# MarToonLi/StableDiffusionEO

Hardware: AMD Instinct MI355X
Metric: 512x512 canny2image images/sec (20 DDIM steps); ms per UNet step reported alongside (higher is better)
Workload: dtype f16; 1 GPU; SD1.5 + ControlNet-canny 512x512, batch=1 per GPU (CFG pair fused, N=2), 20 DDIM steps + VAE decode, fp16 storage / fp32 accumulate (BASELINE configs[1]); model_config=sd15, ddim_steps=20, parallelism=dp1 (image index -> rank, RCCL all_gather of final latents), weights=seeded synthetic (no checkpoint in the container)

## Files before the change

### stablediffusioneo_amd/csrc/api_ops.hip

```cpp
#include <stdarg.h>

#include "../../include/sdeo.h"
#include "sdeo_internal.h"
#include "kernels.h"

namespace sdeo {

static thread_local std::string g_last_error;

void set_error(const std::string& msg) { g_last_error = msg; }

int fail(const char* fmt, ...) {
  char buf[1024];
  va_list ap;
  va_start(ap, fmt);
  vsnprintf(buf, sizeof(buf), fmt, ap);
  va_end(ap);
  g_last_error = buf;
  return 1;
}

}

using namespace sdeo;
// ... 112 lines not shown
  return 0;
}

int sdeo_conv2d_nhwc_f16(void* y, const void* x, const void* w_krsc, const float* bias, const float* bias2, const void* res,
                         int n, int h, int w, int cin, int cout, int ksize, int stride, int upsample2x, int act, float scale,
                         void* workspace, size_t workspace_bytes, void* stream) {
  const Fp8Arm arm = disarm_fp8();
  ConvGemm p;
  if (int rc = fill_conv(p, n, h, w, cin, cout, ksize, stride, upsample2x)) return rc;
  p.x = (const f16*)x; p.w = (const f16*)w_krsc; p.y = (f16*)y; p.bias = bias; p.bias2 = bias2; p.res = (const f16*)res;
  p.act = act; p.scale = scale; p.workspace = (float*)workspace; p.workspace_bytes = workspace_bytes;
  take_fp8(p, arm);
  return conv_gemm(p, S(stream));
}

size_t sdeo_conv2d_pad_workspace_bytes(int n, int h, int w, int cin, int cout, int ksize, int stride, int upsample2x, int pad_before,
                                       int pad_after) {
  ConvGemm p;
  if (fill_conv(p, n, h, w, cin, cout, ksize, stride, upsample2x, pad_before, pad_after)) return 0;
  return conv_gemm_workspace_bytes(p);
}

int sdeo_conv2d_pad_nhwc_f16(void* y, const void* x, const void* w_krsc, const float* bias, const float* bias2, const void* res,
                             int n, int h, int w, int cin, int cout, int ksize, int stride, int upsample2x, int pad_before, int pad_after,
                             int act, float scale, void* workspace, size_t workspace_bytes, void* stream) {
  const Fp8Arm arm = disarm_fp8();
  SDEO_CHECK(pad_before >= 0 && pad_after >= 0, "conv2d_pad: negative padding (%d, %d)", pad_before, pad_after);
  ConvGemm p;
  if (int rc = fill_conv(p, n, h, w, cin, cout, ksize, stride, upsample2x, pad_before, pad_after)) return rc;
  p.x = (const f16*)x; p.w = (const f16*)w_krsc; p.y = (f16*)y; p.bias = bias; p.bias2 = bias2; p.res = (const f16*)res;
// ... 196 lines not shown
```

### stablediffusioneo_amd/csrc/conv_gemm.hip

```cpp
#include <stdlib.h>

#include <array>
#include <map>

#include <type_traits>
#include <utility>

#include "conv_inl.h"

namespace sdeo {

template <int BM, int BN, int STAGES, bool UPS, bool WS, bool W8 = false, int KPB = 1, bool MX = false>
__global__ __launch_bounds__(WS ? 512 : 256) void conv_gemm_dma_kernel(const KP pp) {
  kernarg_warm<sizeof(KP)>();
  KP pl = pp;
  asm volatile("" : "+s"(pl.M), "+s"(pl.N), "+s"(pl.K), "+s"(pl.Hi), "+s"(pl.Wi), "+s"(pl.Cin), "+s"(pl.Wo),
               "+s"(pl.S), "+s"(pl.stride), "+s"(pl.pad), "+s"(pl.HoWo), "+s"(pl.ldx), "+s"(pl.ldw), "+s"(pl.nk),
               "+s"(pl.nk_per_split), "+s"(pl.tiles_m), "+s"(pl.tiles_n), "+s"(pl.n_fastest));
  const KP& p = pl;
  static_assert(!MX || (WS && !W8 && !UPS && KPB == 1), "the block-scaled fp8 path exists for the plain wave-specialised GEMM");
  constexpr int BK = 64, RPP = 32;
  constexpr int WRPP = W8 ? 64 : 32;
  constexpr int XP = BM / RPP, WP = (BN + WRPP - 1) / WRPP, L = XP + WP;
  constexpr int TM = BM / 2, TN = BN / 2, MI = TM / 16, NI = TN / 16;
// ... 137 lines not shown
  };
  const int ngroups = (nk + KPB - 1) / KPB;

  if constexpr (WS) {
    if (!do_mma) {
      if (nk > 0) {
#pragma unroll
        for (int s = 0; s < PF; ++s)
          if (s < nk) issue(s);
        for (int g = 0; g < ngroups; ++g) {
          retire(g);
          __builtin_amdgcn_s_barrier();
          refill(g);
        }
      }
      __builtin_amdgcn_s_barrier();
      return;
    }
  }

  const int frow = lane & 15, fq = lane >> 4;
  constexpr int g0 = 0;
  f32x4 acc[NI][MI];
#pragma unroll
  for (int i = 0; i < NI; ++i)
#pragma unroll
    for (int j = 0; j < MI; ++j) acc[i][j] = f32x4{0.f, 0.f, 0.f, 0.f};

  float2* lnsm = reinterpret_cast<float2*>(smem + STAGES * STAGE);
  const bool ln_lds = p.ln_stats != nullptr && p.splitk == 1;
// ... 212 lines not shown
  stamp(p, 3);
  if (dbg_on(p, 32)) return;
  static_assert(4 * epilogue_scratch_bytes(TN) <= STAGES * STAGE, "epilogue scratch");
  constexpr int SCR = (STAGES * STAGE / 4) & ~15;
  constexpr int NBLK = epilogue_blocks(TN, MI, SCR);
  char* scratch = smem + wave * SCR;
  epilogue<NI, MI, TM, TN, NBLK>(pe, acc, m0, n0, wm, wn, frow, fq, z, bpre, use_bpre, scratch, ln_lds ? lnsm + wm * TM : nullptr);
  if (pe.gn_out) {
    asm volatile("s_waitcnt lgkmcnt(0)" ::: "memory");
    __builtin_amdgcn_s_barrier();
    if (wm == 0) {
      const int bimg = m0 / pe.HoWo;
      gn_partials_finish<TN, 2>(pe, smem + 2 * wn * SCR, SCR, lane, bimg, (m0 - bimg * pe.HoWo) / BM, n0 + wn * TN);
    }
  }
  if (dbg_on(p, 64)) {
    stamp(p, 4);
    asm volatile("s_waitcnt vmcnt(0)" ::: "memory");
    stamp(p, 5);
  }
}

template <int BM, int BN, int BK, bool GENERIC>
__global__ __launch_bounds__(256) void conv_gemm_kernel(const KP pp) {
  kernarg_warm<sizeof(KP)>();
  const KP& p = pp;
  constexpr int CPR = BK / 8;
  constexpr int RPP = 256 / CPR;
  constexpr int XP = BM / RPP;
  constexpr int WP = BN / RPP;
// ... 132 lines not shown
#pragma unroll
        for (int i = 0; i < NI; ++i)
#pragma unroll
          for (int j = 0; j < MI; ++j)
            acc[i][j] = __builtin_amdgcn_mfma_f32_16x16x32_f16(wf[i], xf[j], acc[i][j], 0, 0, 0);
      }
      if (more) store_tile(cur ^ 1);
      __syncthreads();
    }
  }
  f32x4 nob[NI];
#pragma unroll
  for (int i = 0; i < NI; ++i) nob[i] = f32x4{0.f, 0.f, 0.f, 0.f};
  static_assert(4 * epilogue_scratch_bytes(TN) <= 2 * STAGE, "epilogue scratch");
  epilogue<NI, MI, TM, TN>(p, acc, m0, n0, wm, wn, frow, fq, z, nob, false, smem + wave * epilogue_scratch_bytes(TN));
}

__global__ __launch_bounds__(256) void splitk_reduce_kernel(const KP pp) {
  kernarg_warm<sizeof(KP)>();
  KP pl = pp;
  asm volatile("" : "+s"(pl.M), "+s"(pl.N), "+s"(pl.HoWo), "+s"(pl.ldy), "+s"(pl.ldres), "+s"(pl.ld_bias2), "+s"(pl.act),
               "+s"(pl.bias_per_row), "+s"(pl.splitk), "+s"(pl.res_rows));
  const KP& p = pl;
  const int64_t idx = (int64_t)blockIdx.x * 256 + threadIdx.x;
  const int n4 = p.N / 4;
  if (idx >= (int64_t)p.M * n4) return;
  const int m = (int)(idx / n4);
  const int n = (int)(idx - (int64_t)m * n4) * 4;
  f32x4 v = f32x4{0.f, 0.f, 0.f, 0.f};
  const float* src = p.ws + (size_t)m * p.N + n;
  const size_t zs = (size_t)p.M * p.N;
  f32x4 bv = f32x4{0.f, 0.f, 0.f, 0.f}, b2 = bv;
  f16x4 rv = f16x4{0, 0, 0, 0};
  if (p.bias) {
    if (p.bias_per_row) bv += p.bias[m];
    else bv = *reinterpret_cast<const f32x4*>(p.bias + n);
  }
  if (p.bias2) b2 = *reinterpret_cast<const f32x4*>(p.bias2 + (size_t)(m / p.HoWo) * p.ld_bias2 + n);
  if (p.res) rv = *reinterpret_cast<const f16x4*>(p.res + (size_t)res_row(p, m) * p.ldres + n);
  for (int z0 = 0; z0 < p.splitk; z0 += 8) {
    f32x4 t[8];
// ... 20 lines not shown
  } else if (p.act == 4) {
#pragma unroll
    for (int t = 0; t < 4; ++t) v[t] = fmaxf(v[t], 0.f);
  }
  v *= p.scale;
#pragma unroll
  for (int t = 0; t < 4; ++t) v[t] += (float)rv[t];
  if (p.y32) {
    *reinterpret_cast<f32x4*>(p.y32 + (size_t)m * p.ldy + n) = v;
  } else {
    f16x4 o;
#pragma unroll
    for (int t = 0; t < 4; ++t) o[t] = (f16)v[t];
    *reinterpret_cast<f16x4*>(p.y + (size_t)m * p.ldy + n) = o;
  }
}

template <typename K>
static int launch_k(K kernel, int smem, DeviceOnce* attr_done, const KP& kp, int tiles, hipStream_t stream, int threads = 256) {
  if (attr_done->need()) {
    SDEO_HIP(hipFuncSetAttribute(reinterpret_cast<const void*>(kernel), hipFuncAttributeMaxDynamicSharedMemorySize, smem));
    attr_done->mark();
  }
  hipLaunchKernelGGL(kernel, dim3(tiles, 1, kp.splitk), dim3(threads), smem, stream, kp);
  SDEO_HIP(hipGetLastError());
  return 0;
}

template <int BM, int BN, int ST, bool UPS, bool WS, bool W8 = false, int KPB = 1, bool MX = false>
static int launch_dma(const KP& kp, int tiles, hipStream_t stream) {
// ... 236 lines not shown
               "conv_gemm: fp8 weights need Cin %% 64 == 0 (Cin=%d), no folded upsample and 16-byte aligned rows (ldw=%d bytes)", p.Cin, p.ldw);
  pl = make_plan(p);
  SDEO_CHECK(!p.wscale || (kTiles[pl.tile].caps & CAP_W8), "conv_gemm: no fp8-weight plan for this shape");
  SDEO_CHECK(!p.mx_sx || (kTiles[pl.tile].caps & CAP_MX), "conv_gemm: no block-scaled fp8 plan for this shape");
  SDEO_CHECK(p.act != 3 || (pl.splitk == 1 && (kTiles[pl.tile].bn / 2) % 32 == 0), "conv_gemm: no GEGLU-capable plan");
  kp = KP{};
  kp.x = p.x; kp.w = p.w; kp.y = p.y; kp.y32 = p.y32; kp.bias = p.bias; kp.bias2 = p.bias2; kp.res = p.res;
  kp.ws = p.workspace;
  kp.M = p.M; kp.N = p.N; kp.K = p.K;
  kp.Hi = p.Hi; kp.Wi = p.Wi; kp.Cin = p.Cin; kp.Ho = p.Ho; kp.Wo = p.Wo; kp.S = p.S; kp.stride = p.stride; kp.pad = p.pad;
  kp.ups = p.ups; kp.HoWo = p.Ho * p.Wo;
  kp.ldx = p.ldx; kp.ldw = p.ldw; kp.ldy = p.ldy; kp.ldres = p.ldres; kp.ld_bias2 = p.ld_bias2;
  kp.res_rows = p.res_rows > 0 ? p.res_rows : p.M;
  kp.act = p.act; kp.bias_per_row = p.bias_per_row; kp.scale = p.scale;
  kp.wscale = p.wscale;
  if (p.mx_sx) {
    SDEO_CHECK(p.mx_sw && p.R == 1 && p.S == 1 && p.stride == 1 && !p.ups && !p.wscale && p.Cin % 64 == 0 && !p.bias_per_row,
               "conv_gemm: block-scaled fp8 operands go with a plain GEMM whose K is a multiple of 128");
    SDEO_CHECK(p.mx_ldsx >= p.K / 16 && p.mx_ldsw >= p.K / 16, "conv_gemm: scale rows too short (%d, %d < %d)", p.mx_ldsx, p.mx_ldsw, p.K / 16);
    kp.mx_sx = p.mx_sx; kp.mx_sw = p.mx_sw; kp.mx_ldsx = p.mx_ldsx; kp.mx_ldsw = p.mx_ldsw;
  }
  if (p.ln_stats) {
    SDEO_CHECK(p.ln_s && p.ln_strips >= 1 && p.ln_ld >= p.ln_strips && p.ln_c > 0, "conv_gemm: incomplete LayerNorm-fold arguments");
    SDEO_CHECK(!p.bias_per_row && !p.y32, "conv_gemm: the LayerNorm fold applies to row-major fp16 products only");
    kp.ln_stats = p.ln_stats; kp.ln_s = p.ln_s; kp.ln_strips = p.ln_strips; kp.ln_ld = p.ln_ld;
    kp.ln_invc = 1.0f / (float)p.ln_c; kp.ln_eps = p.ln_eps;
  }
  if (p.stats_out) {
    const int strips = pl.splitk == 1 ? cdiv(p.N, plan_tn(pl)) : 0;
    SDEO_CHECK(strips >= 1 && p.stats_ld >= strips && p.y && !p.y32 && p.act != 3,
// ... 19 lines not shown
    static const int epi = [] { const char* e = getenv("SDEO_EPI_COALESCE"); return e ? atoi(e) : 1; }();
    kp.coalesce = epi && p.y && !p.y32 && pl.splitk == 1 && !p.bias_per_row && p.N % (p.act == 3 ? 16 : 8) == 0 && p.ldy % 8 == 0 &&
                  (reinterpret_cast<uintptr_t>(p.y) & 15) == 0 &&
                  (!p.res || (p.ldres % 8 == 0 && (reinterpret_cast<uintptr_t>(p.res) & 15) == 0));
    SDEO_CHECK(!p.gn_out || kp.coalesce, "conv_gemm: GroupNorm partials need the LDS-transposed epilogue");
  }
  if (pl.splitk > 1) {
    const size_t need = (size_t)pl.splitk * p.M * p.N * sizeof(float);
    SDEO_CHECK(p.workspace && p.workspace_bytes >= need, "conv_gemm: split-K workspace too small (%zu < %zu)",
               p.workspace_bytes, need);
  }
  if (kTiles[pl.tile].kind == TK_HALO) SDEO_CHECK(halo_ok(p, kTiles[pl.tile]), "conv_gemm: halo plan on an ineligible problem");
  return 0;
}

static int dispatch(const Plan& pl, int ups, bool w8, const KP& kp, hipStream_t stream) {
  if (pl.tile < 0 || pl.tile >= kTileCount) return fail("conv_gemm: bad tile %d", pl.tile);
  const TileCfg& c = kTiles[pl.tile];
  const TileLaunch launch = kp.mx_sx ? c.mx : w8 ? c.w8 : ups ? c.ups : c.plain;
  if (!launch) return fail("conv_gemm: tile %d has no %s instantiation", pl.tile, kp.mx_sx ? "block-scaled fp8" : w8 ? "fp8-weight" : "folded-upsample");
  if (int rc = launch(kp, pl.tiles_m * pl.tiles_n, stream)) return rc;
  if (pl.splitk > 1) {
    const int64_t n = (int64_t)kp.M * (kp.N / 4);
    hipLaunchKernelGGL(splitk_reduce_kernel, dim3((unsigned)cdiv64(n, 256)), dim3(256), 0, stream, kp);
    SDEO_HIP(hipGetLastError());
  }
  return 0;
}

int conv_gemm(const ConvGemm& p0, hipStream_t stream) {
  if (p0.mx_sx)
    SDEO_CHECK(p0.K % 128 == 0 && p0.ldx % 16 == 0 && p0.ldw % 16 == 0 && p0.K == p0.Cin, "conv_gemm: block-scaled fp8 GEMM needs K %% 128 == 0 (K=%d, ldx=%d, ldw=%d)", p0.K, p0.ldx, p0.ldw);
  const ConvGemm p = mx_view(p0);
  Plan pl;
  KP kp{};
  if (int rc = prepare(p, pl, kp)) return rc;
  g_last_tile = pl.tile; g_last_splitk = pl.splitk;
  return dispatch(pl, p.ups, p.wscale != nullptr, kp, stream);
}
// ... 98 lines not shown
```

### stablediffusioneo_amd/csrc/conv_halo.hip

```cpp
#include "conv_inl.h"

namespace sdeo {

constexpr int halo_xbytes(int ph, int pw) { return ((ph + 2) * (pw + 2) + 31) / 32 * 32 * 128; }
constexpr int halo_wbytes(int bn) { return (bn + 31) / 32 * 32 * 128; }
constexpr int halo_stages(int ph, int pw, int bn, int tpb = 1) {
  const int s = (160 * 1024 - 2 * halo_xbytes(ph, pw)) / (tpb * halo_wbytes(bn));
  const int cap = tpb == 1 ? 8 : 4;
  return s > cap ? cap : s;
}

template <int PH, int PW, int BN, int NMW, int TPB = 1>
__global__ __launch_bounds__(NMW * 64 + 256) void conv3x3_halo_kernel(const KP pp) {
  kernarg_warm<sizeof(KP)>();
  KP pl = pp;
  asm volatile("" : "+s"(pl.M), "+s"(pl.N), "+s"(pl.Hi), "+s"(pl.Wi), "+s"(pl.Cin), "+s"(pl.ldx), "+s"(pl.ldw),
               "+s"(pl.nk_per_split), "+s"(pl.tiles_m), "+s"(pl.tiles_n));
  const KP& p = pl;
  constexpr int BM = PH * PW;
  constexpr int MI = BM / (16 * NMW), NI = BN / 16;
  constexpr int HWD = PW + 2, XREAL = (PH + 2) * HWD;
  constexpr int LXW = (XREAL + 31) / 32;
  constexpr int XBYTES = LXW * 32 * 128;
  constexpr int LW = (BN + 31) / 32;
// ... 91 lines not shown
      const bool xin = tap >= 1 && tap <= PF - 1 && cr + 1 < ncr;
      if (a == PF - 1) {
        if (xin) wait_vmcnt<(PF - 1) * LWS + LXW>();
        else wait_vmcnt<(PF - 1) * LWS>();
      } else {
        static_for<PF - 1>([&](auto A) {
          if (a == A.value) wait_vmcnt<A.value * LWS>();
        });
      }
      __builtin_amdgcn_s_barrier();
      if (dbg_on(p, 8)) { if (++tap == SPS) { tap = 0; ++cr; } continue; }
      if (tap == 0 && cr + 1 < ncr) issue_x((cr + 1) & 1);
      if (it + PF < lsteps) issue_w((it + PF) % WST);
      if (++tap == SPS) { tap = 0; ++cr; }
    }
    __builtin_amdgcn_s_barrier();
    return;
  }

  const int wave = wave_all;
  const int frow = lane & 15, fq = lane >> 4;
  f32x4 acc[NI][MI];
#pragma unroll
  for (int i = 0; i < NI; ++i)
#pragma unroll
    for (int j = 0; j < MI; ++j) acc[i][j] = f32x4{0.f, 0.f, 0.f, 0.f};

  constexpr bool BPRE = NI <= 5;
  f32x4 bpre[NI];
  const bool use_bpre = BPRE && p.bias && !p.bias_per_row && p.splitk == 1;
// ... 148 lines not shown
```

### stablediffusioneo_amd/csrc/conv_inl.h

```cpp
#pragma once
#include <utility>

#include "kernels.h"

namespace sdeo {

struct KP {
  const f16* x;
  const f16* w;
  f16* y;
  float* y32;
  const float* bias;
  const float* bias2;
  const f16* res;
  float* ws;
  int M, N, K;
  int Hi, Wi, Cin, Ho, Wo, S, stride, pad, ups;
  int HoWo;
  int ldx, ldw, ldy, ldres, ld_bias2;
  int res_rows;
  int act, bias_per_row;
  float scale;
  int nk, nk_per_split, splitk;
  int tiles_m, tiles_n;
  int dbg;
  int n_fastest;
  int coalesce;
  const float* ln_stats;
  const float* ln_s;
  int ln_strips, ln_ld;
  float ln_invc, ln_eps;
  const float* wscale;
  float* stats_out;
  int stats_ld;
  float* gn_out;
  int gn_cpg, gn_slots, gn_groups;
  const unsigned char* mx_sx;
  const unsigned char* mx_sw;
  int mx_ldsx, mx_ldsw;
};

#ifdef SDEO_DEBUG_KERNELS
__device__ __forceinline__ bool dbg_on(const KP& p, int bit) { return (p.dbg & bit) != 0; }
#else
__device__ __forceinline__ constexpr bool dbg_on(const KP&, int) { return false; }
#endif

constexpr int kStampWGs = 4096, kStampSlots = 16;
static __device__ unsigned long long g_stamps[kStampWGs * kStampSlots];
__device__ __forceinline__ void stamp_cycles(const KP& p, int slot) {
  if (dbg_on(p, 64) && threadIdx.x == 0) {
    const int wg = blockIdx.x + gridDim.x * blockIdx.z;
    if (wg < kStampWGs) g_stamps[wg * kStampSlots + slot] = __builtin_amdgcn_s_memtime();
  }
}
__device__ __forceinline__ void stamp(const KP& p, int slot) {
  if (dbg_on(p, 64) && threadIdx.x == 0) {
    const int wg = blockIdx.x + gridDim.x * blockIdx.z;
    if (wg < kStampWGs) g_stamps[wg * kStampSlots + slot] = __builtin_amdgcn_s_memrealtime();
  }
}

static __device__ __attribute__((aligned(256))) const unsigned int g_zero_page[64] = {0};

template <int BK>
__device__ __forceinline__ int swz_chunk(int row, int chunk) {
  if (BK == 64) return chunk ^ ((row >> 1) & 7);
  return chunk ^ (((row >> 3) & 1) * 3);
}

constexpr int epilogue_scratch_bytes(int tn) { return 16 * (tn * 4 + 16) + 32 * tn; }

__device__ __forceinline__ unsigned long long pin_u64(unsigned long long v) {
  unsigned lo = __builtin_amdgcn_readfirstlane((unsigned)v), hi = __builtin_amdgcn_readfirstlane((unsigned)(v >> 32));
  asm volatile("" : "+s"(lo), "+s"(hi));
// ... 464 lines not shown
```

### stablediffusioneo_amd/csrc/handle_common.h

```cpp
#pragma once
#include <stdlib.h>

#include <algorithm>
#include <functional>
#include <string>
#include <unordered_map>
#include <vector>

#include "kernels.h"

namespace sdeo {

static inline size_t align_up(size_t v, size_t a) { return (v + a - 1) / a * a; }

enum WKind { W_CONV, W_LINEAR, W_VEC, W_GEGLU_W, W_GEGLU_B };
struct WEntry {
  std::string name;
  int64_t dims[4];
  int ndim;
  WKind kind;
  size_t off;
  int ipad;
  bool loaded;
};

struct WeightStore {
  std::vector<WEntry> entries;
  std::unordered_map<std::string, int> index;
  size_t size = 0;
  char* slab = nullptr;
  size_t slab_bytes = 0;
  float* stage = nullptr;
  size_t stage_bytes = 0;

  size_t take(size_t bytes) {
    const size_t off = align_up(size, 256);
    size = off + bytes;
    return off;
  }
  void add(const std::string& name, WKind kind, std::initializer_list<int64_t> dims, size_t off, int ipad = 0) {
    WEntry w{name, {1, 1, 1, 1}, (int)dims.size(), kind, off, ipad, false};
    int i = 0;
    for (auto d : dims) w.dims[i++] = d;
    index[name] = (int)entries.size();
    entries.push_back(w);
  }
  const WEntry* find(const std::string& name) const {
    auto it = index.find(name);
    return it == index.end() ? nullptr : &entries[it->second];
  }
  template <class T>
  const T* ptr(const std::string& name) const { return reinterpret_cast<const T*>(slab + entries[index.at(name)].off); }

// ... 55 lines not shown

  int require_all(const char* who) {
    std::string missing;
    int nmiss = 0;
    for (auto& w : entries)
      if (!w.loaded) {
        if (nmiss < 5) missing += (nmiss ? ", " : "") + w.name;
        ++nmiss;
      }
    SDEO_CHECK(nmiss == 0, "%s: %d tensors missing (%s%s)", who, nmiss, missing.c_str(), nmiss > 5 ? ", ..." : "");
    if (stage) { (void)hipFree(stage); stage = nullptr; }
    return 0;
  }
};

struct Op {
  std::function<int(hipStream_t)> fn;
  const char* key = "other";
  std::string tag;
  double flops = 0, bytes = 0;
  bool zero_conv = false;
  template <class F>
  Op(F f, const char* key_ = "other", double flops_ = 0, double bytes_ = 0, std::string tag_ = std::string())
      : fn(std::move(f)), key(key_), tag(std::move(tag_)), flops(flops_), bytes(bytes_) {}
  int operator()(hipStream_t s) const { return fn(s); }
};
typedef std::vector<Op> Program;

struct Profiler {
  struct Rec { std::string key; double flops, bytes; hipEvent_t a, b; };
  bool on = false;
  std::vector<Rec> recs;
  std::string report;

  void begin() {
    for (auto& r : recs) { (void)hipEventDestroy(r.a); (void)hipEventDestroy(r.b); }
    recs.clear();
    on = true;
  }
  int record(const Op& op, hipStream_t s) {
    static const bool detail = [] { const char* v = getenv("SDEO_PROFILE_DETAIL"); return v && atoi(v) != 0; }();
    Rec r{detail && !op.tag.empty() ? std::string(op.key) + " | " + op.tag : std::string(op.key), op.flops, op.bytes, nullptr, nullptr};
// ... 49 lines not shown
```

### stablediffusioneo_amd/csrc/kernels.h

```cpp
#pragma once
#include "common.h"

namespace sdeo {

struct ConvGemm {
  const f16* x = nullptr;
  const f16* w = nullptr;
  f16* y = nullptr;
  float* y32 = nullptr;
  const float* bias = nullptr;
  const float* bias2 = nullptr;
  const f16* res = nullptr;
  float* workspace = nullptr;
  size_t workspace_bytes = 0;
  int M = 0, N = 0, K = 0;
  int B = 1, Hi = 1, Wi = 1, Cin = 0;
  int Ho = 1, Wo = 1, R = 1, S = 1, stride = 1, pad = 0;
  int pad_after = -1;
  int ups = 0;
  int ldx = 0, ldw = 0, ldy = 0, ldres = 0, ld_bias2 = 0;
  int act = 0;
  int bias_per_row = 0;
  float scale = 1.0f;
  int force_tile = -1;
// ... 1 lines not shown
  const float* ln_stats = nullptr;
  const float* ln_s = nullptr;
  int ln_strips = 0, ln_ld = 0;
  int ln_c = 0;
  float ln_eps = 1e-5f;
  const float* wscale = nullptr;
  float* stats_out = nullptr;
  int stats_ld = 0;
  float* gn_out = nullptr;
  int gn_cpg = 0, gn_slots = 0, gn_groups = 0;
  const uint8_t* mx_sx = nullptr;
  const uint8_t* mx_sw = nullptr;
  int mx_ldsx = 0, mx_ldsw = 0;
  int res_rows = 0;
  int plan_B = 0;
};
int conv_gemm(const ConvGemm& p, hipStream_t stream);
inline int conv_pad_after(const ConvGemm& p) { return p.pad_after < 0 ? p.pad : p.pad_after; }
int conv_gemm_gn_slots(const ConvGemm& p, int cpg);
bool conv_gemm_plan_is_halo(const ConvGemm& p);
int conv_gemm_stats_strips(const ConvGemm& p);
int conv_gemm_read_stamps(unsigned long long* out, int n);
int conv_halo_read_stamps(unsigned long long* out, int n);
size_t conv_gemm_workspace_bytes(const ConvGemm& p);
int conv_gemm_plan_splitk(const ConvGemm& p);
void conv_gemm_query_plan(const ConvGemm& p, int key[10], int* tile, int* splitk);
void conv_gemm_last_plan(int* tile, int* splitk);
int conv_gemm_tile_info(int tile, int* kind, int* bm, int* bn, int* stages, int* caps, const char** name);
const char* conv_gemm_kernel_name(const ConvGemm& p);
void conv_gemm_debug_force(int tile, int splitk);
// ... 84 lines not shown
```

### stablediffusioneo_amd/csrc/net.hip

```cpp
#include <functional>
#include <memory>
#include <unordered_map>
#include <vector>

#include "../../include/sdeo.h"
#include "handle_common.h"

using namespace sdeo;

namespace {

static inline int round8(int c) { return (c + 7) / 8 * 8; }

const char* NS_UNET = "model.diffusion_model.";
const char* NS_CN = "control_model.";
const char* NS_VAE = "first_stage_model.";

enum BlkKind { B_CONV_IN, B_RES, B_ATTN, B_DOWN, B_UP };
struct Blk { BlkKind kind; std::string name; int cin, cout; };
struct UPlan {
  std::vector<std::vector<Blk>> in, out;
  std::vector<Blk> mid;
  std::vector<int> in_ch, in_ds;
};
// ... 179 lines not shown
  bool use_control = true;
  static constexpr int kTabRows = 128;
  float* emb_all[2] = {nullptr, nullptr};
  float* temb_tab[2] = {nullptr, nullptr};
  int64_t* tab_t = nullptr;
  int tab_count = 0;
  const float* emb_cur[2] = {nullptr, nullptr};
  int emb_ld_cur[2] = {0, 0};
  T x0;
  T eps16;
  Program p_hint, p_ctx_cn, p_ctx_unet, p_cn, p_cn_export, p_ctrl_import, p_unet_enc, p_unet_dec, p_unet_noctrl, p_vae, p_vae_enc;
  Program p_temb[2], p_temb_tab, p_x0, p_eps_export, p_unet_dec_fused;
  Program p_unet_enc_sh, p_cn_sh;
  std::vector<size_t> ctrl_elems;
  size_t device_bytes = 0;
  bool autotune = false;
  Profiler prof;
};

namespace {

typedef sdeo_handle_s Engine;

struct Registry {
  Engine* e;
  bool quant = true;
  void region(size_t off, int rows, int cols) {
    if (!quant) return;
    e->qindex[off] = (int)e->qregions.size();
    e->qregions.push_back(QRegion{off, rows, cols, 0, 0});
// ... 264 lines not shown
  }

  const WEntry* W(const std::string& name) {
    const WEntry* w = e->ws.find(name);
    if (!w && err.empty()) err = "unknown weight " + name;
    return w;
  }
  const f16* wptr(const std::string& name) { return W(name) ? e->ws.ptr<f16>(name) : nullptr; }
  const float* vptr(const std::string& name) { return W(name) ? e->ws.ptr<float>(name) : nullptr; }
  const f16* named_w(const std::string& name) { return reinterpret_cast<const f16*>(e->ws.slab + e->named_off.at(name)); }
  const float* named_v(const std::string& name) { return reinterpret_cast<const float*>(e->ws.slab + e->named_off.at(name)); }


  void launch_conv(ConvGemm p, const float* scale_host, RowStats* stats = nullptr, T* gn_y = nullptr, const ConvOpts* lo = nullptr) {
    const int Mplan = p.plan_B ? p.M / p.B * p.plan_B : p.M;
    if (e->act_bits == 8 && e->mxslab && Mplan >= e->mx_min_rows && p.R == 1 && p.S == 1 && p.stride == 1 && !p.ups && p.K % 128 == 0 &&
        p.K == p.Cin && p.ldx % 16 == 0 && !p.bias_per_row && p.y && !p.y32) {
      auto it = e->mxindex.find((size_t)(reinterpret_cast<const char*>(p.w) - e->ws.slab));
      if (it != e->mxindex.end() && it->second.cols == p.ldw && p.N <= it->second.rows) {
        T xq = alloc2d(Mplan, p.K / 2), xs = alloc2d(Mplan, (p.K / 32 + 15) / 16 * 8);
        uint8_t* q = reinterpret_cast<uint8_t*>(xq.p);
        uint8_t* sc = reinterpret_cast<uint8_t*>(xs.p);
        const int lds = (p.K / 32 + 15) / 16 * 16;
        const f16* xp = p.x; const int M_ = p.M, K_ = p.K, ldx_ = p.ldx;
        push([=](hipStream_t s) { return quantize_mx(q, sc, xp, M_, K_, ldx_, K_, lds, s); }, "quantize_mx", 0, 3.0 * M_ * K_,
             "rows" + std::to_string(M_) + " C" + std::to_string(K_));
        p.x = reinterpret_cast<const f16*>(q); p.ldx = p.K;
        p.w = reinterpret_cast<const f16*>(e->mxslab + it->second.q_off); p.ldw = it->second.cols;
        p.mx_sx = sc; p.mx_ldsx = lds;
        p.mx_sw = reinterpret_cast<const uint8_t*>(e->mxslab + it->second.s_off); p.mx_ldsw = it->second.cols / 32;
        if (!dry && !share) ++e->mx_launches;
        mx_tmp.push_back(xq); mx_tmp.push_back(xs);
      }
    }
    if (!p.mx_sx && e->weight_bits == 8 && Mplan <= 512 && p.Cin % 64 == 0 && !p.ups && !p.bias_per_row && !conv_gemm_plan_is_halo(p)) {
      auto it = e->qindex.find((size_t)(reinterpret_cast<const char*>(p.w) - e->ws.slab));
      if (it != e->qindex.end()) {
        const QRegion& q = e->qregions[it->second];
        if (q.cols == p.ldw && p.N <= q.rows) {
          p.w = reinterpret_cast<const f16*>(e->q8slab + q.q_off);
          p.wscale = reinterpret_cast<const float*>(e->q8slab + q.s_off);
        }
      }
    }
    max_splitk = std::max(max_splitk, e->autotune ? conv_gemm_autotune_workspace_bytes(p) : conv_gemm_workspace_bytes(p));
    if (!dry && e->autotune && !share) {
      ConvGemm q = p;
      q.workspace = ws_sel ? e->splitk_ws2 : e->splitk_ws;
      q.workspace_bytes = e->splitk_ws_bytes;
      if (conv_gemm_autotune(q, 0) && err.empty()) err = std::string("autotune failed: ") + sdeo_last_error();
    }
    if (gn_y && gn_y->gnp_off != (size_t)-1) {
      const int cpg = p.N / 32, slots = conv_gemm_gn_slots(p, cpg);
      if (slots > 0) {
        gn_y->gnp = reinterpret_cast<float*>(base + gn_y->gnp_off);
        gn_y->gn_slots = slots;
// ... 3 lines not shown
    if (!dry && !share && getenv("SDEO_DUMP_GEMM"))
      fprintf(stderr, "SDEO_GEMM %d %d %d %d %d %d %d %d %d %d %s\n", p.M, p.N, p.K, p.Cin, p.R, p.stride, p.ups, p.B, p.Hi, p.Wi,
              conv_gemm_kernel_name(p));
    bool stats_by_kernel = false;
    if (stats) {
      stats->c = p.N;
      stats->strips = conv_gemm_stats_strips(p);
      if (stats->strips > 0 && stats->strips <= stats->ld) { p.stats_out = stats->p; p.stats_ld = stats->ld; }
      else { stats->strips = 1; stats_by_kernel = true; }
    }
    Engine* eng = e;
    const int sel = ws_sel;
    const float* const* b2cur = lo ? lo->bias2_cur : nullptr;
    const int* b2ld = lo ? lo->ld_bias2_cur : nullptr;
    const int b2off = lo ? lo->bias2_off : 0;
    push([p, scale_host, eng, sel, b2cur, b2ld, b2off](hipStream_t s) mutable {
      p.workspace = sel ? eng->splitk_ws2 : eng->splitk_ws;
      p.workspace_bytes = eng->splitk_ws_bytes;
      if (scale_host) p.scale = *scale_host;
      if (b2cur) { p.bias2 = *b2cur + b2off; p.ld_bias2 = *b2ld; }
      return conv_gemm(p, s);
    }, conv_gemm_kernel_name(p), 2.0 * p.M * p.N * p.K,
       2.0 * ((double)p.M * p.Cin * (p.R * p.S > 1 ? 1 : 1) + (double)p.N * p.K + (double)p.M * p.N),
       "M" + std::to_string(p.M) + " N" + std::to_string(p.N) + " K" + std::to_string(p.K) + " R" + std::to_string(p.R) + " s" +
           std::to_string(p.stride) + " u" + std::to_string(p.ups));
    for (auto& t : mx_tmp) release(t);
    mx_tmp.clear();
    if (stats_by_kernel) {
      float* sp = stats->p; const int ld = stats->ld, rows = p.M, C = p.N, ldy = p.ldy; const f16* y = p.y;
      push([=](hipStream_t s) { return row_stats(sp, ld, y, ldy, rows, C, s); }, "row_stats", 0, 2.0 * rows * C,
           "rows" + std::to_string(rows) + " C" + std::to_string(C));
    }
  }

  std::vector<T> mx_tmp;
  RowStats alloc_stats(int rows, int c) {
    RowStats st;
    st.ld = std::max(1, (c + 31) / 32);
    st.c = c;
    T raw = alloc2d(rows, st.ld * 4);
// ... 649 lines not shown
    T q = b.conv(mo, std::string(NS_VAE) + "quant_conv", 2 * zc, 1, 1, 0, qo);
    b.release(mo);
    {
      float* zp = e->enc_z; float* mp = e->enc_moments; const float* np_ = e->enc_noise; const int* with_noise = &e->enc_with_noise;
      const f16* in = q.p; const int ld = q.ld, HW = h * w; const float sf = c.vae_scale_factor;
      b.push([=](hipStream_t s) { return vae_posterior(zp, mp, in, ld, *with_noise ? np_ : nullptr, zc, HW, sf, s); }, "vae_posterior", 0,
             (2.0 * 2 * zc + 4.0 * 4 * zc) * HW);
    }
    b.release(q);
  }
  *max_splitk = b.max_splitk;
  *max_gn = b.max_gn;
  *err = b.err;
}

template <typename Tp>
static int dev_alloc(Engine* e, Tp** p, size_t bytes) {
  void* v = nullptr;
  SDEO_HIP(hipMalloc(&v, bytes < 256 ? 256 : bytes));
  e->extra_allocs.push_back(v);
  e->device_bytes += bytes;
  *p = reinterpret_cast<Tp*>(v);
  return 0;
}

static void free_configured(Engine* e) {
  for (void* v : e->extra_allocs) (void)hipFree(v);
  e->extra_allocs.clear();
  if (e->arena) (void)hipFree(e->arena);
  e->arena = nullptr;
// ... 215 lines not shown
  SDEO_HIP(hipMemset(h->arena2, 0, h->arena2_bytes));
  h->device_bytes += h->arena_bytes + h->arena2_bytes;
  if (int rc = dev_alloc(h, &h->splitk_ws, ms)) return rc;
  if (int rc = dev_alloc(h, &h->splitk_ws2, ms)) return rc;
  h->splitk_ws_bytes = ms;
  if (int rc = dev_alloc(h, &h->gn_ws, mg)) return rc;
  if (int rc = dev_alloc(h, &h->gn_ws2, mg)) return rc;
  h->gn_ws_bytes = mg;
  {
    Arena a, a2;
    build_all(h, a, a2, false, &ms, &mg, &err);
    SDEO_CHECK(err.empty(), "sdeo_configure: %s", err.c_str());
    SDEO_CHECK(align_up(a.peak, 256) == h->arena_bytes && align_up(a2.peak, 256) == h->arena2_bytes,
               "sdeo_configure: arena plan not reproducible");
  }
  SDEO_HIP(hipDeviceSynchronize());
  return 0;
}

static int copy_in(void* dst, const void* src, size_t bytes, hipStream_t s) {
  if (dst == src) return 0;
  SDEO_HIP(hipMemcpyAsync(dst, src, bytes, hipMemcpyDeviceToDevice, s));
  return 0;
}

static int stage_inputs(sdeo_handle h, const float* x, const float* hint, const int64_t* t, const float* ctx, int hint_is_new,
                        int ctx_for_net, hipStream_t s) {
  const sdeo_config& c = h->cfg;
  const size_t px = (size_t)h->lh * h->lw;
  if (x) if (int rc = copy_in(h->in_x, x, (size_t)h->N * c.in_channels * px * 4, s)) return rc;
  if (t) if (int rc = copy_in(h->in_t, t, (size_t)h->N * 8, s)) return rc;
  if (hint && hint_is_new) {
// ... 226 lines not shown
```

### stablediffusioneo_amd/csrc/sdeo_internal.h

```cpp
#ifndef SDEO_INTERNAL_H
#define SDEO_INTERNAL_H

#include <stdint.h>

#ifdef __cplusplus
extern "C" {
#endif

void sdeo_debug_force_gemm_plan(int tile, int splitk);
void sdeo_debug_force_gemm_order(int order);
const char* sdeo_debug_conv2d_kernel_name(int n, int h, int w, int cin, int cout, int ksize, int stride, int upsample2x);
const char* sdeo_debug_attention_kernel_name(int B, int H, int Tq, int Tk, int d, int causal);
int sdeo_debug_conv2d_plan(int n, int h, int w, int cin, int cout, int ksize, int stride, int upsample2x, int act, int fp8, int* key10,
                           int* tile, int* splitk);
int sdeo_debug_gemm_plan(int m, int n, int k, int act, int fp8, int* key10, int* tile, int* splitk);
void sdeo_debug_last_gemm_plan(int* tile, int* splitk);
int sdeo_debug_tile_info(int tile, int* kind, int* bm, int* bn, int* stages, int* caps, const char** name);
int sdeo_debug_read_stamps(int which, unsigned long long* out, int n);
int sdeo_debug_silu(void* y, const void* x, int64_t n, void* stream);

int sdeo_debug_fold_layernorm(void* w_out, float* s_out, float* b_out, const void* w, const float* gamma, const float* beta,
                              const float* bias, int rows, int c, void* stream);
int sdeo_debug_compose_proj(void* w_out, float* b_out, const void* wp, const float* bp, const void* w2, const float* b2, int c, int k2,
                            void* stream);
// ... 8 lines not shown

int sdeo_debug_gemm_res_rows_f16(void* y, int ldy, const void* x, int ldx, const void* w, int ldw, const float* bias, const void* res,
                                 int ldres, int res_rows, int m, int n, int k, float* stats, int stats_ld, int* strips_out, void* workspace,
                                 size_t workspace_bytes, void* stream);
int sdeo_debug_attention_qb_f16(void* o, int ldo, const void* q, int ldq, const void* k, int ldk, const void* v, int ldv, int b,
                                int q_batches, int heads, int tq, int tk, int tk_stride, int v_batch_stride, int d, float scale, void* stream);

int sdeo_debug_quantize_mx(void* q_out, void* scales_out, const void* x, int rows, int cols, void* stream);
int sdeo_debug_gemm_mx_f16(void* y, int ldy, const void* xq, const void* xs, const void* wq, const void* ws, const float* bias, const void* res,
                           int ldres, int m, int n, int k, int act, void* workspace, size_t workspace_bytes, void* stream);
int sdeo_debug_quantize_fp8_rows(void* w_f16_inout, void* q_out, float* scale_out, int rows, int cols, void* stream);
void sdeo_debug_next_weights_fp8(const void* q, const float* scale);

int sdeo_debug_mx_launches(sdeo_handle h);

const char* sdeo_debug_fake_scribble_profile(const uint8_t* edges, int h, int w, uint8_t* scribble, float* control_chw, void* workspace,
                                             size_t workspace_bytes, void* stream);

#ifdef __cplusplus
}
#endif
#endif
```

Baseline: 8.441 images/s.

## Prefetch next conv's weights into cache from tail of preceding conv kernels

Each conv/GEMM op in the UNet and ControlNet programs now carries a prefetch range pointing at the weight tensor read by the next weight-reading op. At the end of the conv kernels (producer waves in the wave-specialised path, after the epilogue elsewhere, and in the split-K reduce) the kernel issues strided dword loads across that range so the next layer's weights are warm in L2/MALL. The goal is to hide weight-fetch latency at batch 2, where layers are bandwidth-bound. The cost is extra memory traffic and tail work in every kernel, plus a risk of evicting useful data. It is on by default, can be disabled by environment variable, and is capped at 64MB per range.

New measurement: 8.410 images/s (median of 2 runs). Within noise of the previous version (-0.4%).

```diff
diff --git a/stablediffusioneo_amd/csrc/api_ops.hip b/stablediffusioneo_amd/csrc/api_ops.hip
--- a/stablediffusioneo_amd/csrc/api_ops.hip
+++ b/stablediffusioneo_amd/csrc/api_ops.hip
@@ -150,6 +150,19 @@
   return conv_gemm(p, S(stream));
 }
 
+int sdeo_debug_conv2d_prefetch_f16(void* y, const void* x, const void* w_krsc, const float* bias, const void* res, int n, int h, int w,
+                                   int cin, int cout, int ksize, const void* pf, int pf_bytes, void* workspace, size_t workspace_bytes,
+                                   void* stream) {
+  (void)disarm_fp8();
+  SDEO_CHECK(pf_bytes >= 0 && (pf || pf_bytes == 0), "conv2d_prefetch: a range of %d bytes needs an address", pf_bytes);
+  ConvGemm p;
+  if (int rc = fill_conv(p, n, h, w, cin, cout, ksize, 1, 0)) return rc;
+  p.x = (const f16*)x; p.w = (const f16*)w_krsc; p.y = (f16*)y; p.bias = bias; p.res = (const f16*)res;
+  p.workspace = (float*)workspace; p.workspace_bytes = workspace_bytes;
+  p.pf = (const char*)pf; p.pf_bytes = pf_bytes;
+  return conv_gemm(p, S(stream));
+}
+
 size_t sdeo_conv2d_pad_workspace_bytes(int n, int h, int w, int cin, int cout, int ksize, int stride, int upsample2x, int pad_before,
                                        int pad_after) {
   ConvGemm p;
diff --git a/stablediffusioneo_amd/csrc/conv_gemm.hip b/stablediffusioneo_amd/csrc/conv_gemm.hip
--- a/stablediffusioneo_amd/csrc/conv_gemm.hip
+++ b/stablediffusioneo_amd/csrc/conv_gemm.hip
@@ -175,6 +175,7 @@
           refill(g);
         }
       }
+      prefetch_touch(pp.pf, pp.pf_bytes, wave_u, 4);
       __builtin_amdgcn_s_barrier();
       return;
     }
@@ -417,6 +418,7 @@
       gn_partials_finish<TN, 2>(pe, smem + 2 * wn * SCR, SCR, lane, bimg, (m0 - bimg * pe.HoWo) / BM, n0 + wn * TN);
     }
   }
+  if constexpr (!WS) prefetch_touch<true>(pp.pf, pp.pf_bytes, wave_u, 4);
   if (dbg_on(p, 64)) {
     stamp(p, 4);
     asm volatile("s_waitcnt vmcnt(0)" ::: "memory");
@@ -579,6 +581,7 @@
   for (int i = 0; i < NI; ++i) nob[i] = f32x4{0.f, 0.f, 0.f, 0.f};
   static_assert(4 * epilogue_scratch_bytes(TN) <= 2 * STAGE, "epilogue scratch");
   epilogue<NI, MI, TM, TN>(p, acc, m0, n0, wm, wn, frow, fq, z, nob, false, smem + wave * epilogue_scratch_bytes(TN));
+  prefetch_touch(p.pf, p.pf_bytes, __builtin_amdgcn_readfirstlane(wave), 4);
 }
 
 __global__ __launch_bounds__(256) void splitk_reduce_kernel(const KP pp) {
@@ -589,7 +592,8 @@
   const KP& p = pl;
   const int64_t idx = (int64_t)blockIdx.x * 256 + threadIdx.x;
   const int n4 = p.N / 4;
-  if (idx >= (int64_t)p.M * n4) return;
+  do {
+  if (idx >= (int64_t)p.M * n4) break;
   const int m = (int)(idx / n4);
   const int n = (int)(idx - (int64_t)m * n4) * 4;
   f32x4 v = f32x4{0.f, 0.f, 0.f, 0.f};
@@ -640,6 +644,8 @@
     for (int t = 0; t < 4; ++t) o[t] = (f16)v[t];
     *reinterpret_cast<f16x4*>(p.y + (size_t)m * p.ldy + n) = o;
   }
+  } while (false);
+  prefetch_touch(p.pf, p.pf_bytes, __builtin_amdgcn_readfirstlane(threadIdx.x >> 6), 4);
 }
 
 template <typename K>
@@ -906,6 +912,9 @@
   kp.res_rows = p.res_rows > 0 ? p.res_rows : p.M;
   kp.act = p.act; kp.bias_per_row = p.bias_per_row; kp.scale = p.scale;
   kp.wscale = p.wscale;
+  SDEO_CHECK(p.pf_bytes >= 0 && (p.pf_bytes == 0 || p.pf) && (reinterpret_cast<uintptr_t>(p.pf) & 3) == 0,
+             "conv_gemm: prefetch range must be 4-byte aligned and non-negative (%d bytes)", p.pf_bytes);
+  kp.pf = p.pf_bytes > 0 ? p.pf : nullptr; kp.pf_bytes = p.pf_bytes;
   if (p.mx_sx) {
     SDEO_CHECK(p.mx_sw && p.R == 1 && p.S == 1 && p.stride == 1 && !p.ups && !p.wscale && p.Cin % 64 == 0 && !p.bias_per_row,
                "conv_gemm: block-scaled fp8 operands go with a plain GEMM whose K is a multiple of 128");
@@ -955,15 +964,21 @@
   return 0;
 }
 
-static int dispatch(const Plan& pl, int ups, bool w8, const KP& kp, hipStream_t stream) {
+static int dispatch(const Plan& pl, int ups, bool w8, const KP& kp0, hipStream_t stream) {
   if (pl.tile < 0 || pl.tile >= kTileCount) return fail("conv_gemm: bad tile %d", pl.tile);
+  KP kp = kp0, kr = kp0;
+  if (pl.splitk > 1 && kp0.pf) {
+    const int head = (kp0.pf_bytes / 2) & ~127;
+    kp.pf_bytes = head;
+    kr.pf = kp0.pf + head; kr.pf_bytes = kp0.pf_bytes - head;
+  }
   const TileCfg& c = kTiles[pl.tile];
   const TileLaunch launch = kp.mx_sx ? c.mx : w8 ? c.w8 : ups ? c.ups : c.plain;
   if (!launch) return fail("conv_gemm: tile %d has no %s instantiation", pl.tile, kp.mx_sx ? "block-scaled fp8" : w8 ? "fp8-weight" : "folded-upsample");
   if (int rc = launch(kp, pl.tiles_m * pl.tiles_n, stream)) return rc;
   if (pl.splitk > 1) {
     const int64_t n = (int64_t)kp.M * (kp.N / 4);
-    hipLaunchKernelGGL(splitk_reduce_kernel, dim3((unsigned)cdiv64(n, 256)), dim3(256), 0, stream, kp);
+    hipLaunchKernelGGL(splitk_reduce_kernel, dim3((unsigned)cdiv64(n, 256)), dim3(256), 0, stream, kr);
     SDEO_HIP(hipGetLastError());
   }
   return 0;
diff --git a/stablediffusioneo_amd/csrc/conv_halo.hip b/stablediffusioneo_amd/csrc/conv_halo.hip
--- a/stablediffusioneo_amd/csrc/conv_halo.hip
+++ b/stablediffusioneo_amd/csrc/conv_halo.hip
@@ -129,6 +129,7 @@
       if (it + PF < lsteps) issue_w((it + PF) % WST);
       if (++tap == SPS) { tap = 0; ++cr; }
     }
+    prefetch_touch(pp.pf, pp.pf_bytes, lw, 4);
     __builtin_amdgcn_s_barrier();
     return;
   }
diff --git a/stablediffusioneo_amd/csrc/conv_inl.h b/stablediffusioneo_amd/csrc/conv_inl.h
--- a/stablediffusioneo_amd/csrc/conv_inl.h
+++ b/stablediffusioneo_amd/csrc/conv_inl.h
@@ -38,6 +38,8 @@
   const unsigned char* mx_sx;
   const unsigned char* mx_sw;
   int mx_ldsx, mx_ldsw;
+  const char* pf;
+  int pf_bytes;
 };
 
 #ifdef SDEO_DEBUG_KERNELS
@@ -59,6 +61,22 @@
     const int wg = blockIdx.x + gridDim.x * blockIdx.z;
     if (wg < kStampWGs) g_stamps[wg * kStampSlots + slot] = __builtin_amdgcn_s_memrealtime();
   }
+}
+
+template <bool DRAIN = false>
+__device__ __forceinline__ void prefetch_touch(const char* pf, int pf_bytes, int wave, int nwaves) {
+  if (pf == nullptr || pf_bytes < 4) return;
+  if (DRAIN) __builtin_amdgcn_s_waitcnt(0x0f70);
+  const unsigned bytes = (unsigned)pf_bytes;
+  const unsigned nlines = (bytes + 127u) >> 7, last = (bytes - 4u) & ~3u;
+  const unsigned wg = blockIdx.x + gridDim.x * blockIdx.z;
+  const unsigned stride = gridDim.x * gridDim.z * (unsigned)nwaves * 64u;
+  unsigned sink = 0;
+  for (unsigned i = (wg * (unsigned)nwaves + (unsigned)wave) * 64u + (threadIdx.x & 63u); i < nlines; i += stride) {
+    const unsigned off = min(i << 7, last);
+    asm volatile("global_load_dword %0, %1, %2" : "+v"(sink) : "v"(off), "s"(pf));
+  }
+  asm volatile("" ::"v"(sink));
 }
 
 static __device__ __attribute__((aligned(256))) const unsigned int g_zero_page[64] = {0};
diff --git a/stablediffusioneo_amd/csrc/handle_common.h b/stablediffusioneo_amd/csrc/handle_common.h
--- a/stablediffusioneo_amd/csrc/handle_common.h
+++ b/stablediffusioneo_amd/csrc/handle_common.h
@@ -4,6 +4,7 @@
 #include <algorithm>
 #include <functional>
 #include <string>
+#include <type_traits>
 #include <unordered_map>
 #include <vector>
 
@@ -33,10 +34,18 @@
   float* stage = nullptr;
   size_t stage_bytes = 0;
 
+  std::vector<std::pair<size_t, size_t>> blocks;
   size_t take(size_t bytes) {
     const size_t off = align_up(size, 256);
     size = off + bytes;
+    blocks.push_back({off, bytes});
     return off;
+  }
+  const std::pair<size_t, size_t>* block_of(size_t off) const {
+    auto it = std::upper_bound(blocks.begin(), blocks.end(), off, [](size_t o, const std::pair<size_t, size_t>& b) { return o < b.first; });
+    if (it == blocks.begin()) return nullptr;
+    --it;
+    return off < it->first + it->second ? &*it : nullptr;
   }
   void add(const std::string& name, WKind kind, std::initializer_list<int64_t> dims, size_t off, int ipad = 0) {
     WEntry w{name, {1, 1, 1, 1}, (int)dims.size(), kind, off, ipad, false};
@@ -122,18 +131,48 @@
   }
 };
 
+struct WeightRead {
+  const char* p = nullptr;
+  size_t bytes = 0;
+  size_t tensor_off = 0;
+  size_t tensor_bytes = 0;
+};
+struct Prefetch { const char* p = nullptr; int bytes = 0; };
+
 struct Op {
-  std::function<int(hipStream_t)> fn;
+  std::function<int(hipStream_t, const Prefetch&)> fn;
+  bool carrier = false;
+  WeightRead wread;
+  Prefetch pf;
+  int pf_target = -1;
   const char* key = "other";
   std::string tag;
   double flops = 0, bytes = 0;
   bool zero_conv = false;
   template <class F>
   Op(F f, const char* key_ = "other", double flops_ = 0, double bytes_ = 0, std::string tag_ = std::string())
-      : fn(std::move(f)), key(key_), tag(std::move(tag_)), flops(flops_), bytes(bytes_) {}
-  int operator()(hipStream_t s) const { return fn(s); }
+      : key(key_), tag(std::move(tag_)), flops(flops_), bytes(bytes_) {
+    if constexpr (std::is_invocable_v<F&, hipStream_t, const Prefetch&>) fn = std::move(f);
+    else fn = [f = std::move(f)](hipStream_t s, const Prefetch&) mutable { return f(s); };
+  }
+  int operator()(hipStream_t s) const { return fn(s, pf); }
 };
 typedef std::vector<Op> Program;
+
+static inline void wire_prefetch(Program& p, bool on, size_t cap) {
+  Prefetch next;
+  int target = -1;
+  for (int i = (int)p.size() - 1; i >= 0; --i) {
+    Op& op = p[i];
+    op.pf = (on && op.carrier) ? next : Prefetch();
+    op.pf_target = op.pf.p ? target : -1;
+    if (op.wread.p) {
+      const size_t n = std::min(std::min(op.wread.bytes, cap), (size_t)0x7fffff80);
+      next.p = n >= 4 ? op.wread.p : nullptr; next.bytes = n >= 4 ? (int)n : 0;
+      target = i;
+    }
+  }
+}
 
 struct Profiler {
   struct Rec { std::string key; double flops, bytes; hipEvent_t a, b; };
diff --git a/stablediffusioneo_amd/csrc/kernels.h b/stablediffusioneo_amd/csrc/kernels.h
--- a/stablediffusioneo_amd/csrc/kernels.h
+++ b/stablediffusioneo_amd/csrc/kernels.h
@@ -39,6 +39,8 @@
   int mx_ldsx = 0, mx_ldsw = 0;
   int res_rows = 0;
   int plan_B = 0;
+  const char* pf = nullptr;
+  int pf_bytes = 0;
 };
 int conv_gemm(const ConvGemm& p, hipStream_t stream);
 inline int conv_pad_after(const ConvGemm& p) { return p.pad_after < 0 ? p.pad : p.pad_after; }
diff --git a/stablediffusioneo_amd/csrc/net.hip b/stablediffusioneo_amd/csrc/net.hip
--- a/stablediffusioneo_amd/csrc/net.hip
+++ b/stablediffusioneo_amd/csrc/net.hip
@@ -1,9 +1,12 @@
+#include <string.h>
+
 #include <functional>
 #include <memory>
 #include <unordered_map>
 #include <vector>
 
 #include "../../include/sdeo.h"
+#include "sdeo_internal.h"
 #include "handle_common.h"
 
 using namespace sdeo;
@@ -217,6 +220,7 @@
   Program p_unet_enc_sh, p_cn_sh;
   std::vector<size_t> ctrl_elems;
   size_t device_bytes = 0;
+  bool prefetch_on = true;
   bool autotune = false;
   Profiler prof;
 };
@@ -511,6 +515,16 @@
 
   void launch_conv(ConvGemm p, const float* scale_host, RowStats* stats = nullptr, T* gn_y = nullptr, const ConvOpts* lo = nullptr) {
     const int Mplan = p.plan_B ? p.M / p.B * p.plan_B : p.M;
+    WeightRead wread;
+    if (const char* w0 = reinterpret_cast<const char*>(p.w); e->ws.slab && w0 >= e->ws.slab && w0 < e->ws.slab + e->ws.slab_bytes) {
+      wread.tensor_off = (size_t)(w0 - e->ws.slab);
+      if (const auto* blk = e->ws.block_of(wread.tensor_off)) {
+        wread.p = w0;
+        wread.bytes = ((size_t)(p.N - 1) * p.ldw + p.K) * 2;
+        wread.tensor_bytes = blk->first + blk->second - wread.tensor_off;
+        if (wread.bytes > wread.tensor_bytes) wread = WeightRead();
+      }
+    }
     if (e->act_bits == 8 && e->mxslab && Mplan >= e->mx_min_rows && p.R == 1 && p.S == 1 && p.stride == 1 && !p.ups && p.K % 128 == 0 &&
         p.K == p.Cin && p.ldx % 16 == 0 && !p.bias_per_row && p.y && !p.y32) {
       auto it = e->mxindex.find((size_t)(reinterpret_cast<const char*>(p.w) - e->ws.slab));
@@ -526,6 +540,8 @@
         p.w = reinterpret_cast<const f16*>(e->mxslab + it->second.q_off); p.ldw = it->second.cols;
         p.mx_sx = sc; p.mx_ldsx = lds;
         p.mx_sw = reinterpret_cast<const uint8_t*>(e->mxslab + it->second.s_off); p.mx_ldsw = it->second.cols / 32;
+        wread.p = e->mxslab + it->second.q_off;
+        wread.bytes = wread.tensor_bytes = it->second.s_off + (size_t)it->second.rows * (it->second.cols / 32) - it->second.q_off;
         if (!dry && !share) ++e->mx_launches;
         mx_tmp.push_back(xq); mx_tmp.push_back(xs);
       }
@@ -537,6 +553,8 @@
         if (q.cols == p.ldw && p.N <= q.rows) {
           p.w = reinterpret_cast<const f16*>(e->q8slab + q.q_off);
           p.wscale = reinterpret_cast<const float*>(e->q8slab + q.s_off);
+          wread.p = e->q8slab + q.q_off;
+          wread.bytes = wread.tensor_bytes = q.s_off + (size_t)q.rows * 4 - q.q_off;
         }
       }
     }
@@ -570,16 +588,18 @@
     const float* const* b2cur = lo ? lo->bias2_cur : nullptr;
     const int* b2ld = lo ? lo->ld_bias2_cur : nullptr;
     const int b2off = lo ? lo->bias2_off : 0;
-    push([p, scale_host, eng, sel, b2cur, b2ld, b2off](hipStream_t s) mutable {
+    push([p, scale_host, eng, sel, b2cur, b2ld, b2off](hipStream_t s, const Prefetch& pf) mutable {
       p.workspace = sel ? eng->splitk_ws2 : eng->splitk_ws;
       p.workspace_bytes = eng->splitk_ws_bytes;
       if (scale_host) p.scale = *scale_host;
       if (b2cur) { p.bias2 = *b2cur + b2off; p.ld_bias2 = *b2ld; }
+      p.pf = pf.p; p.pf_bytes = pf.bytes;
       return conv_gemm(p, s);
     }, conv_gemm_kernel_name(p), 2.0 * p.M * p.N * p.K,
        2.0 * ((double)p.M * p.Cin * (p.R * p.S > 1 ? 1 : 1) + (double)p.N * p.K + (double)p.M * p.N),
        "M" + std::to_string(p.M) + " N" + std::to_string(p.N) + " K" + std::to_string(p.K) + " R" + std::to_string(p.R) + " s" +
            std::to_string(p.stride) + " u" + std::to_string(p.ups));
+    if (!dry) { prog->back().carrier = true; prog->back().wread = wread; }
     for (auto& t : mx_tmp) release(t);
     mx_tmp.clear();
     if (stats_by_kernel) {
@@ -1259,6 +1279,11 @@
   *err = b.err;
 }
 
+static const size_t kPrefetchCap = (size_t)64 << 20;
+static std::vector<Program*> prefetch_programs(Engine* e) {
+  return {&e->p_cn, &e->p_cn_sh, &e->p_unet_enc, &e->p_unet_enc_sh, &e->p_unet_dec, &e->p_unet_dec_fused, &e->p_unet_noctrl};
+}
+
 template <typename Tp>
 static int dev_alloc(Engine* e, Tp** p, size_t bytes) {
   void* v = nullptr;
@@ -1504,8 +1529,51 @@
     SDEO_CHECK(align_up(a.peak, 256) == h->arena_bytes && align_up(a2.peak, 256) == h->arena2_bytes,
                "sdeo_configure: arena plan not reproducible");
   }
+  {
+    const char* sw = getenv("SDEO_WEIGHT_PREFETCH");
+    const char* cap = getenv("SDEO_WEIGHT_PREFETCH_CAP");
+    h->prefetch_on = !sw || atoi(sw) != 0;
+    const size_t cap_bytes = cap && atoll(cap) > 0 ? (size_t)atoll(cap) : kPrefetchCap;
+    for (Program* p : prefetch_programs(h)) wire_prefetch(*p, h->prefetch_on, cap_bytes);
+  }
   SDEO_HIP(hipDeviceSynchronize());
   return 0;
+}
+
+int sdeo_debug_prefetch_ranges(sdeo_handle h, int program_id, sdeo_prefetch_range* out, int cap) {
+  if (!h || !h->arena || program_id < 0 || program_id > 8 || (cap > 0 && !out)) { (void)fail("sdeo_debug_prefetch_ranges: bad arguments"); return -1; }
+  const Program* progs[9] = {&h->p_cn, &h->p_cn_sh, &h->p_unet_enc, &h->p_unet_enc_sh, &h->p_unet_dec, &h->p_unet_dec_fused, &h->p_unet_noctrl,
+                             &h->p_vae, &h->p_vae_enc};
+  const Program& p = *progs[program_id];
+  auto name_of = [&](const WeightRead& w, char* dst, size_t n) {
+    std::string name;
+    const auto* blk = h->ws.block_of(w.tensor_off);
+    if (blk) {
+      size_t best = (size_t)-1;
+      for (auto& en : h->ws.entries)
+        if (en.off >= blk->first && en.off < blk->first + blk->second && en.off < best) { best = en.off; name = en.name; }
+      if (name.empty())
+        for (auto& kv : h->named_off)
+          if (kv.second >= blk->first && kv.second < blk->first + blk->second && kv.second < best) { best = kv.second; name = kv.first; }
+    }
+    snprintf(dst, n, "%s", name.c_str());
+  };
+  for (int i = 0; i < (int)p.size() && i < cap; ++i) {
+    sdeo_prefetch_range& r = out[i];
+    memset(&r, 0, sizeof(r));
+    r.op = i; r.target_op = -1;
+    r.carrier = p[i].carrier ? 1 : 0;
+    if (p[i].wread.p) { r.reads_bytes = (long long)p[i].wread.bytes; r.reads_tensor_bytes = (long long)p[i].wread.tensor_bytes; name_of(p[i].wread, r.reads, sizeof(r.reads)); }
+    if (p[i].pf.p && p[i].pf_target >= 0) {
+      const WeightRead& w = p[p[i].pf_target].wread;
+      r.target_op = p[i].pf_target;
+      r.pf_offset = (long long)(p[i].pf.p - w.p);
+      r.pf_bytes = p[i].pf.bytes;
+      r.tensor_bytes = (long long)w.tensor_bytes;
+      name_of(w, r.tensor, sizeof(r.tensor));
+    }
+  }
+  return (int)p.size();
 }
 
 static int copy_in(void* dst, const void* src, size_t bytes, hipStream_t s) {
diff --git a/stablediffusioneo_amd/csrc/sdeo_internal.h b/stablediffusioneo_amd/csrc/sdeo_internal.h
--- a/stablediffusioneo_amd/csrc/sdeo_internal.h
+++ b/stablediffusioneo_amd/csrc/sdeo_internal.h
@@ -46,6 +46,16 @@
 
 int sdeo_debug_mx_launches(sdeo_handle h);
 
+typedef struct sdeo_prefetch_range {
+  int op, carrier, target_op, pf_bytes;
+  long long pf_offset, tensor_bytes, reads_bytes, reads_tensor_bytes;
+  char tensor[160], reads[160];
+} sdeo_prefetch_range;
+int sdeo_debug_conv2d_prefetch_f16(void* y, const void* x, const void* w_krsc, const float* bias, const void* res, int n, int h, int w,
+                                   int cin, int cout, int ksize, const void* pf, int pf_bytes, void* workspace, size_t workspace_bytes,
+                                   void* stream);
+int sdeo_debug_prefetch_ranges(sdeo_handle h, int program, sdeo_prefetch_range* out, int cap);
+
 const char* sdeo_debug_fake_scribble_profile(const uint8_t* edges, int h, int w, uint8_t* scribble, float* control_chw, void* workspace,
                                              size_t workspace_bytes, void* stream);
 
```
